# do-mpc/do-mpc

Measured on AMD Instinct MI355X. Metric: MPC steps/sec (make_step wall-time), industrial_poly robust multi-stage, higher is better.
Workload: dtype f64

## Files before the change

### do_mpc_amd/csrc/dompc_driver.h

```cpp

DOMPC_DEV inline int epsg_off(const KArgs& A) { return A.node_eps_off[0]; }
DOMPC_DEV inline int epsg_n(const KArgs& A) { return A.n_opt_x - A.node_eps_off[0]; }
DOMPC_DEV inline void epsg_grad(const Thr& T, const Prob& Q) {
  const KArgs& A = *Q.A;
  const int o = epsg_off(A), nv = epsg_n(A);
  for (int j = T.tid; j < nv; j += T.nt) {
    double g = 0.0, r = 0.0;
    for (int e = 0; e < A.n_edges; ++e) {
      const int q = j - (A.node_eps_off[A.edge_parent[e]] - o);
      if (q < 0 || q >= NSE) continue;
      g += Q.sf * DOMPC_EPS_PEN[q];
      const double* yd = Q.lam + A.edge_row0[e] + NW + NX;
      for (int i = 0; i < NE; ++i)
        if (nl_slack(i) == q) r -= yd[i] * Q.sgn[e * NE1 + i];
    }
    Q.gf[o + j] = g;
    Q.rd[o + j] = g + r - Q.zl[o + j] + Q.zu[o + j];
  }
  T.sync();
}
DOMPC_DEV inline double epsg_rowsum(const Prob& Q, int j, const double* v, const double* v0) {
  const KArgs& A = *Q.A;
  const int o = epsg_off(A);
  double t = 0.0;
// ... 10 lines not shown
  const KArgs& A = *Q.A;
  const int o = epsg_off(A);
  for (int e = T.tid; e < A.n_edges; e += T.nt) {
    const int jo = A.node_eps_off[A.edge_parent[e]] - o;
    const int r0 = A.edge_row0[e] + NW + NX;
    for (int i = 0; i < NE; ++i) {
      const int q = nl_slack(i);
      if (q < 0) continue;
      const double ve = v ? v[jo + q] : ((jo + q == j1) ? 1.0 : 0.0);
      Q.c[r0 + i] = Q.ct[r0 + i] - ve * Q.sgn[e * NE1 + i];
    }
  }
  T.sync();
}

DOMPC_DEV inline void solve_problem(const Thr& T, const KArgs& A, int b, int slot) {
  const dompc_options& O = A.opt;
  Prob Q = make_prob(A, slot, A.p + (int64_t)b * A.n_opt_p);
  const double* x0 = A.x0 + (int64_t)b * A.n_opt_x;
  const int nX = A.n_opt_x, nSl = A.n_edges * NE;
  int status = 2, it = 0, n_reg = 0, n_ls_fail = 0, n_sweeps = 0, n_trials = 0, n_soc = 0;

  double cnt[2] = {0.0, 0.0};
  bool singular0;
  {
    double fr[1] = {0.0};
    for (int d = T.tid; d < A.n_dummy; d += T.nt) {
      const int g = A.dummy_idx[d];
      if (!(A.lbx[g] > -INFINITY) && !(A.ubx[g] < INFINITY)) fr[0] += 1.0;
    }
    const int ops[1] = {R_SUM};
    wg_reduce(T, fr, ops);
// ... 247 lines not shown
    if (KAPPA_D != 0.0) bs[0] += KAPPA_D * lin;
    const int ops[1] = {R_SUM};
    wg_reduce(T, bs, ops);
    bar_sum = bs[0];
  }
  int n_filt = 0;
  double delta_last = 0.0;
  int acc_count = 0;
  const double s_max = 100.0;
  double E0 = 0.0;
  int wd_count = 0, wd_iter = 0, n_watchdog = 0;
  bool in_wd = false, wd_resume = false;
  double wd_theta = 0.0, wd_phi = 0.0, wd_dphi = 0.0, wd_alpha = 0.0, wd_amax = 0.0, wd_az = 0.0, wd_delta = 0.0, wd_delta_last = 0.0, wd_bar = 0.0;
  Errs wd_E = E;
  double delta = 0.0, a_max = 1.0, a_z = 1.0, dphi = 0.0;

  while (true) {
    bool skip_first = false;
    if (wd_resume) {
      for (int g = T.tid; g < nX; g += T.nt) { Q.x[g] = Q.x_wd[g]; Q.zl[g] = Q.zl_wd[g]; Q.zu[g] = Q.zu_wd[g]; Q.dx[g] = Q.dx_sv[g]; }
      for (int g = T.tid; g < A.n_g; g += T.nt) { Q.lam[g] = Q.lam_wd[g]; Q.dlam[g] = Q.dlam_sv[g]; }
      for (int g = T.tid; g < nSl; g += T.nt) { Q.s[g] = Q.s_wd[g]; Q.zsl[g] = Q.zsl_wd[g]; Q.zsu[g] = Q.zsu_wd[g]; Q.ds[g] = Q.ds_sv[g]; }
      T.sync();
      E = wd_E; bar_sum = wd_bar; delta = wd_delta; delta_last = wd_delta_last; a_max = wd_amax; a_z = wd_az; dphi = wd_dphi;
      wd_resume = false;
      skip_first = true;
    } else {
    if (bad) { if (in_wd) { bad = 0; wd_resume = true; in_wd = false; wd_count = 0; continue; } status = 3; break; }
    if (T.fget(6)) { status = 6; break; }
    if (((WIDE_OK && T.nwg > 1) || sh_on(A)) && T.fget(7)) { status = 5; break; }
// ... 72 lines not shown
    auto step_rules = [&](double (&r5)[5]) { run_step_rules(T, Q, b, slot, mu, r5); };
    const double theta = E.theta;
    const double phi = E.obj + mu * bar_sum;

    c_t = prof_clock(); g_t = T.gen;
    const double gamma_theta = 1e-5, gamma_phi = 1e-8, eta_phi = 1e-8, s_theta = 1.1, s_phi = 2.3, gamma_alpha = 0.05;
    const double kappa_soc = 0.99;
    double a_min;
    if (dphi < 0.0 && theta <= theta_min)
      a_min = (theta > 0.0) ? gamma_alpha * fmin(gamma_theta, fmin(gamma_phi * theta / (-dphi),
                                                                    pow(theta, s_theta) / pow(-dphi, s_phi)))
                            : gamma_alpha * gamma_theta;
    else if (dphi < 0.0) a_min = gamma_alpha * fmin(gamma_theta, gamma_phi * theta / (-dphi));
    else a_min = gamma_alpha * gamma_theta;
    a_min = fmax(a_min, 1e-14);
    auto eval_trial = [&](double al, double& obj_o, double& th_o, double& bar_o) {
      run_eval_trial(T, Q, b, slot, al, obj_o, th_o, bar_o);
      ++n_trials;
    };
    auto acceptable_ref = [&](double th_, double ph_, double al, bool& armijo_case, double theta, double phi, double dphi) -> bool {
      armijo_case = false;
      bool ok = (ph_ == ph_) && (th_ == th_) && fabs(ph_) < INFINITY && th_ <= theta_max;
      if (ok) {
        for (int q = 0; q < n_filt; ++q)
          if (th_ >= T.filt[2 * q] && ph_ >= T.filt[2 * q + 1]) { ok = false; break; }
      }
      if (ok) {
        const bool switching = dphi < 0.0 && al * pow(-dphi, s_phi) > pow(theta, s_theta);
        const double eps_m = 10.0 * 2.220446049250313e-16 * fabs(phi);
        if (theta <= theta_min && switching) {
          armijo_case = true;
          ok = (ph_ - phi - eps_m <= eta_phi * al * dphi);
// ... 22 lines not shown
    double alpha = skip_first ? 0.5 * a_max : a_max;
    bool accepted = false, armijo_used = false, stale = false;
    double th_t = 0.0, obj_t = 0.0, bar_t = bar_sum;
    int n_ls = skip_first ? 1 : 0;
    bool wd_done = false, wd_augment_ref = false, wd_no_augment = false;
    if (O.watchdog_shortened_iter_trigger > 0 && !in_wd && !skip_first && wd_count >= O.watchdog_shortened_iter_trigger) {
      in_wd = true; wd_iter = 0; ++n_watchdog;
      for (int g = T.tid; g < nX; g += T.nt) { Q.x_wd[g] = Q.x[g]; Q.zl_wd[g] = Q.zl[g]; Q.zu_wd[g] = Q.zu[g]; Q.dx_sv[g] = Q.dx[g]; }
      for (int g = T.tid; g < A.n_g; g += T.nt) { Q.lam_wd[g] = Q.lam[g]; Q.dlam_sv[g] = Q.dlam[g]; }
      for (int g = T.tid; g < nSl; g += T.nt) { Q.s_wd[g] = Q.s[g]; Q.zsl_wd[g] = Q.zsl[g]; Q.zsu_wd[g] = Q.zsu[g]; Q.ds_sv[g] = Q.ds[g]; }
      T.sync();
      wd_E = E; wd_bar = bar_sum; wd_delta = delta; wd_delta_last = delta_last; wd_amax = a_max; wd_az = a_z;
      wd_theta = theta; wd_phi = phi; wd_dphi = dphi; wd_alpha = a_max;
    }
    if (in_wd) {
      eval_trial(alpha, obj_t, th_t, bar_t);
      bool armijo_case = false;
      if (acceptable_ref(th_t, obj_t + mu * bar_t, wd_alpha, armijo_case, wd_theta, wd_phi, wd_dphi)) {
        accepted = true; armijo_used = armijo_case; wd_done = true; wd_augment_ref = true;
        in_wd = false; wd_count = 0;
      } else {
        ++wd_iter;
        const double ph_ = obj_t + mu * bar_t;
        if (wd_iter > O.watchdog_trial_iter_max || !(ph_ == ph_) || !(th_t == th_t) || !(fabs(ph_) < INFINITY)) {
          wd_resume = true; in_wd = false; wd_count = 0;
          continue;
        }
        accepted = true; wd_done = true; wd_no_augment = true;
      }
    }
    while (!wd_done) {
      eval_trial(alpha, obj_t, th_t, bar_t);
      stale = false;
      bool armijo_case = false;
      if (acceptable(th_t, obj_t + mu * bar_t, alpha, armijo_case)) { accepted = true; armijo_used = armijo_case; break; }
      if (n_ls == 0 && O.max_soc > 0 && th_t >= theta) {
        double th_old = theta;
        keep_direction(false);
        soc_residual(alpha);
        bool soc_ok = false;
        for (int k = 0; k < O.max_soc; ++k) {
          ++n_soc; ++n_sweeps;
          if (run_sweep(T, Q, b, slot, mu, 1, delta)) break;
          if (run_backward(T, Q, b, slot, mu, delta)) break;
          run_forward(T, Q, b, slot, mu, delta);
          if (EPS_GLOBAL && epsg_apply(delta, Q.dlam)) break;
          double q5[5];
          step_rules(q5);
          const double a_s = (q5[0] > tau) ? tau / q5[0] : 1.0;
          double obj_s = 0.0, th_s = 0.0, bar_s = 0.0;
          eval_trial(a_s, obj_s, th_s, bar_s);
          bool arm_s = false;
          if (acceptable(th_s, obj_s + mu * bar_s, a_s, arm_s)) {
            accepted = true; armijo_used = arm_s; soc_ok = true;
            alpha = a_s;
            a_z = (q5[1] > tau) ? tau / q5[1] : 1.0;
            obj_t = obj_s; th_t = th_s; bar_t = bar_s;
            break;
          }
          if (!(th_s <= kappa_soc * th_old)) break;
          th_old = th_s;
          soc_residual(a_s);
        }
        if (soc_ok) break;
        keep_direction(true);
        stale = true;
      }
      if (!(alpha * 0.5 >= a_min)) break;
      alpha *= 0.5;
      ++n_ls;
    }
    if (bad) { if (in_wd) { bad = 0; wd_resume = true; in_wd = false; wd_count = 0; continue; } status = 3; break; }
    if (!accepted && stale) eval_trial(alpha, obj_t, th_t, bar_t);
    if (!wd_done) wd_count = n_ls > 0 ? wd_count + 1 : 0;
    if (!accepted) {
      ++n_ls_fail;
      n_filt = 0;
    } else if (!armijo_used && !wd_no_augment) {
      if (T.ltid == 0) {
        int q = n_filt < MAX_FILTER ? n_filt : MAX_FILTER - 1;
        T.filt[2 * q] = (1.0 - gamma_theta) * (wd_augment_ref ? wd_theta : theta);
        T.filt[2 * q + 1] = (wd_augment_ref ? wd_phi : phi) - gamma_phi * (wd_augment_ref ? wd_theta : theta);
      }
      if (n_filt < MAX_FILTER) ++n_filt;
      T.lsync();
    }
    bar_sum = bar_t;
    c_ls += prof_clock() - c_t; g_ls += T.gen - g_t;
    c_t = prof_clock(); g_t = T.gen;
    const Comp Cp = run_accept(T, Q, b, slot, alpha, a_z, mu);
    if (A.trace && b == 0 && T.tid == 0 && it < A.trace_cap) {
      double* tr = A.trace + 8 * it;
      tr[0] = it; tr[1] = mu; tr[2] = E0; tr[3] = E.e_p; tr[4] = E.e_d; tr[5] = accepted ? alpha : -alpha;
      tr[6] = delta; tr[7] = E.obj / Q.sf;
    }
    if (T.tid == 0) T.fset(6, abort_requested(A));
    T.sync();
    c_acc += prof_clock() - c_t; g_acc += T.gen - g_t;
    ++it;
    c_t = prof_clock(); g_t = T.gen; bad = run_sweep(T, Q, b, slot, mu, 0, singular0 ? delta_after(delta_last) : 0.0); c_sweep += prof_clock() - c_t; g_sweep += T.gen - g_t;
    ++n_sweeps;
    if (EPS_GLOBAL) epsg_grad(T, Q);
    if (KAPPA_D != 0.0) Q.mu = mu;
    c_t = prof_clock(); g_t = T.gen; E = measure(T, Q, &Cp); c_meas += prof_clock() - c_t; g_meas += T.gen - g_t;
  }

  if (A.trace && b == 0 && T.tid == 0 && A.trace_cap > 8) { double* tr = A.trace + 8 * (A.trace_cap - 1); tr[0] = (double)c_sweep; tr[1] = (double)c_bwd; tr[2] = (double)c_fwd; tr[3] = (double)c_ls; tr[4] = (double)c_meas; tr[5] = (double)(prof_clock() - c_start); tr[6] = (double)c_ftb; tr[7] = (double)c_acc; if (T.prof) { double* t2 = A.trace + 8 * (A.trace_cap - 2); for (int i = 0; i < 8; ++i) t2[i] = (double)T.prof[i]; double* t3 = A.trace + 8 * (A.trace_cap - 3); for (int i = 0; i < 8; ++i) t3[i] = (double)T.prof[8 + i]; double* t4 = A.trace + 8 * (A.trace_cap - 4); for (int i = 0; i < 8; ++i) t4[i] = (double)T.prof[16 + i]; if (A.trace_cap > 12) { double* t5 = A.trace + 8 * (A.trace_cap - 5); for (int i = 0; i < 8; ++i) t5[i] = (double)T.prof[24 + i]; double* t6 = A.trace + 8 * (A.trace_cap - 6); t6[0] = g_sweep; t6[1] = g_bwd; t6[2] = g_fwd; t6[3] = g_ls; t6[4] = g_meas; t6[5] = T.gen - g_start; t6[6] = g_ftb; t6[7] = g_acc; } } }
  const double isf = 1.0 / Q.sf;
  if (A.x_out) for (int g = T.tid; g < nX; g += T.nt) A.x_out[(int64_t)b * nX + g] = sh_cnt(A, mk_x(A, g)) ? Q.x[g] : 0.0;
  if (A.lam_x_out) for (int g = T.tid; g < nX; g += T.nt) A.lam_x_out[(int64_t)b * nX + g] = sh_cnt(A, mk_x(A, g)) ? (Q.zu[g] - Q.zl[g]) * isf : 0.0;
  if (A.lam_g_out) for (int r = T.tid; r < A.n_g; r += T.nt) A.lam_g_out[(int64_t)b * A.n_g + r] = sh_cnt(A, mk_g(A, r)) ? Q.lam[r] * isf : 0.0;
  if (A.lam_g_out && NE > 0) {
    T.sync();
    for (int g = T.tid; g < nSl; g += T.nt) {
      const int e = g / NE1, i = g % NE1;
      if (!sh_cnt(A, mk_e(A, e))) continue;
      const int row = A.edge_row0[e] + NW + NX + i;
      A.lam_g_out[(int64_t)b * A.n_g + row] = Q.lam[row] * Q.sgn[e * NE1 + i] * isf;
    }
  }
  if (A.g_out) {
// ... 112 lines not shown
```

### do_mpc_amd/csrc/dompc_kernel.h

```cpp
#pragma once
#include <math.h>
#include <stdint.h>
#ifndef DOMPC_HOST_EMU
#include <utility>
#endif
#include "dompc_kargs.h"

namespace dompc {

#ifndef DOMPC_HOST_EMU
#define DOMPC_PHASE __device__ inline
#else
#define DOMPC_PHASE static inline
#endif

constexpr int NX = DOMPC_NX, NU = DOMPC_NU, NP = DOMPC_NP, NTVP = DOMPC_NTVP;
#ifndef DOMPC_EPS_GLOBAL
#define DOMPC_EPS_GLOBAL 0
#endif
constexpr bool EPS_GLOBAL = DOMPC_EPS_GLOBAL != 0 && DOMPC_NS > 0 && DOMPC_NE > 0;
constexpr int NS = EPS_GLOBAL ? 0 : DOMPC_NS;
constexpr int NSE = DOMPC_NS;
constexpr int NVG_MAX = 32;
constexpr int NZ = DOMPC_NZ;
// ... 107 lines not shown
constexpr int ND_P = 0;
constexpr int ND_PV = ND_P + NA * NA;
constexpr int ND_K = ND_PV + NA;
constexpr int ND_KV = ND_K + NV * NA;
constexpr int ND_DXT = ND_KV + NV;
constexpr int ND_AT = ND_DXT + NA;
constexpr int AT_LEN = FREE_ROOT ? 1 + NX + NX * NX : 0;
constexpr int ND_SIZE = ((ND_AT + AT_LEN + 7) / 8) * 8;

struct WsLayout {
  int64_t x, zl, zu, lb, ub, dx, gf, rd, xt, dx_sv;
  int64_t lam, dlam, c, ct, dlam_sv;
  int64_t s, zsl, zsu, sl, su, ds, st, ds_sv;
  int64_t ew, es, nd, mo, gsc, total;
  int64_t x_wd, zl_wd, zu_wd, lam_wd, s_wd, zsl_wd, zsu_wd, dlam_e, sgn;
};

DOMPC_HD inline WsLayout ws_layout(int n_opt_x, int n_g, int n_edges, int e_pad, int n_nodes) {
  WsLayout L;
  int64_t o = 0;
  auto take = [&](int64_t n) { int64_t r = o; o += (n + 7) & ~int64_t(7); return r; };
  L.x = take(n_opt_x); L.zl = take(n_opt_x); L.zu = take(n_opt_x); L.lb = take(n_opt_x); L.ub = take(n_opt_x);
  L.dx = take(n_opt_x); L.gf = take(n_opt_x); L.rd = take(n_opt_x); L.xt = take(n_opt_x);
  L.dx_sv = take(n_opt_x);
  L.lam = take(n_g); L.dlam = take(n_g); L.c = take(n_g); L.ct = take(n_g); L.dlam_sv = take(n_g);
  int64_t nsl = (int64_t)n_edges * NE1;
  L.s = take(nsl); L.zsl = take(nsl); L.zsu = take(nsl); L.sl = take(nsl); L.su = take(nsl);
  L.ds = take(nsl); L.st = take(nsl); L.ds_sv = take(nsl);
  L.ew = take((int64_t)EW_SIZE * e_pad);
  L.es = take((int64_t)ES_SIZE * n_edges);
  L.nd = take((int64_t)ND_SIZE * n_nodes);
  L.mo = take((int64_t)MO_REC * n_edges);
  L.gsc = take(EPS_GLOBAL ? NVG_MAX * (NVG_MAX + 4) : 0);
  L.x_wd = take(n_opt_x); L.zl_wd = take(n_opt_x); L.zu_wd = take(n_opt_x); L.lam_wd = take(n_g);
  L.s_wd = take(nsl); L.zsl_wd = take(nsl); L.zsu_wd = take(nsl);
  L.dlam_e = take(EPS_GLOBAL ? n_g : 0);
  L.sgn = take(nsl);
  o += 256;
  L.total = o;
  return L;
}

#ifndef DOMPC_HOST_EMU
typedef __attribute__((address_space(3))) double ldsd;
#else
typedef double ldsd;
#endif

struct XCtx {
  int on, rank, world;
  double* xbuf;
  volatile uint32_t *req, *ack, *cnt;
// ... 307 lines not shown
    for (int l = 0; l < k; ++l) t += A[i * sai + l * sal] * B[l * sbl + j * sbj];
    D[i * ldd + j] = (beta == 0.0) ? t : beta * D[i * ldd + j] + t;
  }
#endif
}

struct Prob {
  const KArgs* A;
  const double* P;
  double *x, *zl, *zu, *lb, *ub, *dx, *gf, *rd, *xt, *dx_sv;
  double *lb_own, *ub_own;
  double *lam, *dlam, *c, *ct, *dlam_sv;
  double *s, *zsl, *zsu, *sl, *su, *ds, *st, *ds_sv;
  double *ew, *es, *nd, *mo, *gsc;
  double *x_wd, *zl_wd, *zu_wd, *lam_wd, *s_wd, *zsl_wd, *zsu_wd, *dlam_e, *sgn;
  int e_pad;
  double sf;
  double mu;
  int soc;
  double dsw;
  int slot;
  int rp_soc; double rp_mu;
  int lu_ok;
  DOMPC_DEV double& EW(int e, int i) const { return ew[(int64_t)e * EW_SIZE + i]; }
  DOMPC_DEV double* ES(int e) const { return es + (int64_t)e * ES_SIZE; }
  DOMPC_DEV double* ND(int n) const { return nd + (int64_t)n * ND_SIZE; }
  DOMPC_DEV double* MO(int e) const { return mo + (int64_t)e * MO_REC; }
};

DOMPC_DEV inline Prob make_prob(const KArgs& A, int slot, const double* P) {
  WsLayout L = ws_layout(A.n_opt_x, A.n_g, A.n_edges, A.e_pad, A.n_nodes);
  double* w = A.ws + (int64_t)slot * A.ws_stride;
  Prob p;
  p.A = &A; p.P = P;
  p.x = w + L.x; p.zl = w + L.zl; p.zu = w + L.zu; p.lb_own = w + L.lb; p.ub_own = w + L.ub; p.dx = w + L.dx;
  p.lb = A.lb_sh ? A.lb_sh : p.lb_own; p.ub = A.ub_sh ? A.ub_sh : p.ub_own;
  p.gf = w + L.gf; p.rd = w + L.rd; p.xt = w + L.xt; p.dx_sv = w + L.dx_sv;
  p.lam = w + L.lam; p.dlam = w + L.dlam; p.c = w + L.c; p.ct = w + L.ct; p.dlam_sv = w + L.dlam_sv;
  p.s = w + L.s; p.zsl = w + L.zsl; p.zsu = w + L.zsu; p.sl = w + L.sl; p.su = w + L.su;
  p.ds = w + L.ds; p.st = w + L.st; p.ds_sv = w + L.ds_sv;
  p.ew = w + L.ew; p.es = w + L.es; p.nd = w + L.nd; p.mo = w + L.mo; p.gsc = w + L.gsc;
  p.x_wd = w + L.x_wd; p.zl_wd = w + L.zl_wd; p.zu_wd = w + L.zu_wd; p.lam_wd = w + L.lam_wd;
  p.s_wd = w + L.s_wd; p.zsl_wd = w + L.zsl_wd; p.zsu_wd = w + L.zsu_wd; p.dlam_e = w + L.dlam_e; p.sgn = w + L.sgn;
  p.e_pad = A.e_pad; p.sf = 1.0; p.mu = 0.0; p.soc = 0; p.dsw = 0.0; p.slot = slot; p.lu_ok = 1; p.rp_soc = 0; p.rp_mu = 0.0;
  return p;
}
DOMPC_DEV inline void prob_bounds(Prob& Q) {
  const KArgs& A = *Q.A;
  const bool own = (Q.soc & 2) != 0 || !A.lb_sh;
  Q.lb = own ? Q.lb_own : A.lb_sh;
  Q.ub = own ? Q.ub_own : A.ub_sh;
}

DOMPC_DEV constexpr int slot_of(int i, int r) { return i == 0 ? r - 1 : DEG + (i - 1) * (DEG + 1) + r; }
DOMPC_DEV constexpr int next_slot(int i) { return (i + 1 < NI) ? slot_of(i + 1, 0) : M - 1; }

DOMPC_DEV inline int group_index(int tid, int gs) {
#ifndef DOMPC_HOST_EMU
  return __builtin_amdgcn_readfirstlane(tid / gs);
// ... 139 lines not shown
```

### do_mpc_amd/csrc/dompc_phases.h

```cpp

template <bool FINE>
DOMPC_DEV inline double trial_edges(const Thr& T, const Prob& Q) {
  const KArgs& A = *Q.A;
  double f = 0.0;
  if (FINE && !DENSE_EDGE && M > 0) {
    constexpr int NPC = NI * DEG + 1;
    for (int it = T.tid; it < A.n_edges * NPC; it += T.nt) {
      const int e = it % A.n_edges, q = it / A.n_edges;
      const double fe = eval_edge_f_t<true>(Q, e, Q.xt, Q.st, Q.ct, q == 0 ? NI * DEG : q - 1);
      f += fe;
    }
  } else
  for (int e = T.tid; e < A.n_edges; e += T.nt) {
    const int m = mk_e(A, e);
    if (!m) continue;
    const double fe = DENSE_EDGE ? dae_edge_f(Q, e, Q.xt, Q.st, Q.ct) : eval_edge_f(Q, e, Q.xt, Q.st, Q.ct);
    if (sh_cnt(A, m)) f += fe;
  }
  for (int n = T.tid; n < A.n_nodes; n += T.nt)
    if (sh_cnt(A, mk_n(A, n))) f += node_rterm_f(Q, n, Q.xt);
  return f;
}
DOMPC_DEV inline void step_rules_pass(const Thr& T, const Prob& Q, double mu, double (&r5)[5]) {
  const KArgs& A = *Q.A;
// ... 37 lines not shown
      gphi -= mu * r;
    }
    if (u < INFINITY) {
      const double r = fast_rcp(u - sv);
      r5[0] = fmax(r5[0], d * r);
      r5[1] = fmax(r5[1], 1.0 - r * d - mu * r * fast_rcp(Q.zsu[si]));
      gphi += mu * r;
    }
    if (KAPPA_D != 0.0) gphi += KAPPA_D * mu * one_sided(l, u);
    r5[2] += gphi * d;
  }
  const int ops[5] = {R_MAX, R_MAX, R_SUM, R_SUM, R_SUM};
  wg_reduce(T, r5, ops);
}
template <bool FINE>
DOMPC_DEV inline void eval_trial_pass(const Thr& T, const Prob& Q, double al, double& obj_o, double& th_o, double& bar_o) {
  const KArgs& A = *Q.A;
  const int nX = A.n_opt_x, nSl = A.n_edges * NE;
  double r3[3] = {0.0, 0.0, 0.0};
  LogAcc La{1.0, 0, 0};
  double lin = 0.0;
  {
    double x_[DOMPC_FW], d_[DOMPC_FW], l_[DOMPC_FW], u2_[DOMPC_FW];
#define L_(u, g) x_[u] = Q.x[g]; d_[u] = Q.dx[g]; l_[u] = Q.lb[g]; u2_[u] = Q.ub[g];
#define B_(u, g)                                                                               \
    if (mk_x(A, g)) {                                                                      \
      const double xt_ = x_[u] + al * d_[u];                                               \
      Q.xt[g] = xt_;                                                                       \
      if (sh_cnt(A, mk_x(A, g))) {                                                         \
        if (l_[u] > -INFINITY) logacc_add(La, xt_ - l_[u]);                                \
        if (u2_[u] < INFINITY) logacc_add(La, u2_[u] - xt_);                               \
        if (KAPPA_D != 0.0) { const double os_ = one_sided(l_[u], u2_[u]); lin += os_ > 0.0 ? xt_ - l_[u] : (os_ < 0.0 ? u2_[u] - xt_ : 0.0); } \
      }                                                                                    \
    }
    DOMPC_FOR4(nX, L_, B_)
#undef L_
#undef B_
  }
  for (int g = T.tid; g < nSl; g += T.nt) {
    if (!mk_e(A, g / NE1)) continue;
    const int si = (g / NE1) * NE1 + g % NE1;
    Q.st[si] = Q.s[si] + al * Q.ds[si];
  }
  T.sync();
  for (int g = T.tid; g < NX; g += T.nt) Q.ct[g] = FREE_ROOT ? 0.0 : Q.xt[A.node_x_off[0] + g] - Q.P[g] / DOMPC_SX[g];
  if (FREE_ROOT && T.tid == 0) r3[0] += Q.sf * dompc_aterm_f(Q.xt + A.node_x_off[0], Q.P, Q.P + A.p_off_tvp, Q.P + A.p_off_p);
  r3[0] += trial_edges<FINE>(T, Q);
  T.sync();
  {
    double c_[DOMPC_FW];
#define L_(u, g) c_[u] = Q.ct[g];
#define B_(u, g) if (sh_cnt(A, mk_g(A, g))) r3[1] += fabs(c_[u]);
    DOMPC_FOR4(A.n_g, L_, B_)
#undef L_
#undef B_
  }
  for (int g = T.tid; g < nSl; g += T.nt) {
    if (!sh_cnt(A, mk_e(A, g / NE1))) continue;
    const int si = (g / NE1) * NE1 + g % NE1;
    if (Q.sl[si] > -INFINITY) logacc_add(La, Q.st[si] - Q.sl[si]);
    if (Q.su[si] < INFINITY) logacc_add(La, Q.su[si] - Q.st[si]);
    if (KAPPA_D != 0.0) { const double os_ = one_sided(Q.sl[si], Q.su[si]); lin += os_ > 0.0 ? Q.st[si] - Q.sl[si] : (os_ < 0.0 ? Q.su[si] - Q.st[si] : 0.0); }
  }
  r3[2] = -logacc_value(La);
  if (KAPPA_D != 0.0) r3[2] += KAPPA_D * lin;
  const int ops[3] = {R_SUM, R_SUM, R_SUM};
  wg_reduce(T, r3, ops);
  obj_o = r3[0]; th_o = r3[1]; bar_o = r3[2];
}
DOMPC_DEV inline Comp accept_pass(const Thr& T, const Prob& Q, double alpha, double a_z, double mu) {
  const KArgs& A = *Q.A;
  const int nX = A.n_opt_x, nSl = A.n_edges * NE;
  const double ks = 1e10;
  Comp Cp{-INFINITY, INFINITY, 0.0};
  {
    double xt_[DOMPC_FW], x_[DOMPC_FW], d_[DOMPC_FW], l_[DOMPC_FW], u2_[DOMPC_FW], zl_[DOMPC_FW], zu_[DOMPC_FW];
#define L_(u, g) xt_[u] = Q.xt[g]; x_[u] = Q.x[g]; d_[u] = Q.dx[g]; l_[u] = Q.lb[g]; u2_[u] = Q.ub[g]; zl_[u] = Q.zl[g]; zu_[u] = Q.zu[g];
#define B_(u, g)                                                                               \
    if (mk_x(A, g)) {                                                                        \
      const double xv = xt_[u], l = l_[u], ub_ = u2_[u];                                     \
      const bool cnt_ = sh_cnt(A, mk_x(A, g));                                               \
      Q.x[g] = xv;                                                                           \
      if (l > -INFINITY) {                                                                   \
        const double ro = fast_rcp(x_[u] - l);                       \
        const double z = zl_[u] + a_z * (mu * ro - zl_[u] - zl_[u] * ro * d_[u]);            \
        const double dd = xv - l, mr = mu * fast_rcp(dd);                                    \
        const double zn = fmax(fmin(z, ks * mr), mr * (1.0 / ks));                           \
        Q.zl[g] = zn;                                                                        \
        if (cnt_) comp_add(Cp, dd * zn, zn);                                                 \
      }                                                                                      \
      if (ub_ < INFINITY) {                                                                  \
        const double ro = fast_rcp(ub_ - x_[u]);                                             \
        const double z = zu_[u] + a_z * (mu * ro - zu_[u] + zu_[u] * ro * d_[u]);            \
        const double dd = ub_ - xv, mr = mu * fast_rcp(dd);                                  \
        const double zn = fmax(fmin(z, ks * mr), mr * (1.0 / ks));                           \
        Q.zu[g] = zn;                                                                        \
        if (cnt_) comp_add(Cp, dd * zn, zn);                                                 \
      }                                                                                      \
    }
    DOMPC_FOR4(nX, L_, B_)
#undef L_
#undef B_
  }
  for (int g = T.tid; g < nSl; g += T.nt) {
    if (!mk_e(A, g / NE1)) continue;
    const int si = (g / NE1) * NE1 + g % NE1;
    const double sv = Q.st[si], so = Q.s[si], dsv = Q.ds[si];
    const bool cnt_ = sh_cnt(A, mk_e(A, g / NE1));
    Q.s[si] = sv;
    const double l = Q.sl[si], u = Q.su[si];
    if (l > -INFINITY) {
      const double z = Q.zsl[si] + a_z * dz_lo(so, l, Q.zsl[si], dsv, mu);
      const double zn = fmax(fmin(z, ks * mu / (sv - l)), mu / (ks * (sv - l)));
      Q.zsl[si] = zn;
      if (cnt_) comp_add(Cp, (sv - l) * zn, zn);
    }
    if (u < INFINITY) {
      const double z = Q.zsu[si] + a_z * dz_up(so, u, Q.zsu[si], dsv, mu);
      const double zn = fmax(fmin(z, ks * mu / (u - sv)), mu / (ks * (u - sv)));
      Q.zsu[si] = zn;
      if (cnt_) comp_add(Cp, (u - sv) * zn, zn);
    }
  }
  {
    double y_[DOMPC_FW], dy_[DOMPC_FW];
#define L_(u, g) y_[u] = Q.lam[g]; dy_[u] = Q.dlam[g];
#define B_(u, g) if (mk_g(A, g)) Q.lam[g] = y_[u] + alpha * dy_[u];
    DOMPC_FOR4(A.n_g, L_, B_)
#undef L_
#undef B_
  }
  return Cp;
}
struct PhaseRet { unsigned gen, nred, xseq; int rc; };
struct PhaseRet3 { unsigned gen, nred, xseq; double v0, v1, v2; };
#ifndef DOMPC_HOST_EMU
#define DOMPC_PHASE_PROLOGUE                                                        \
  const KArgs A = kernel_args(kp);                                                  \
  Thr T = make_thr(A);                                                              \
  T.kp = kp;                                                                        \
  T.gen = ufl(gen); T.nred = ufl(nred); T.xseq = ufl(xseq);                         \
  Prob Q = make_prob(A, ufl(slot), A.p + (int64_t)ufl(b) * A.n_opt_p);              \
  Q.sf = ufl(sf);
__device__ __attribute__((noinline)) PhaseRet phase_sweep(const void* kp, int b, int slot, double sf, double mu, double dsw, int soc, unsigned gen, unsigned nred, unsigned xseq) {
  DOMPC_PHASE_PROLOGUE
  Q.soc = ufl(soc);
  prob_bounds(Q);
  Q.dsw = ufl(dsw);
  const int rc = sweep<false>(T, Q, ufl(mu));
  return PhaseRet{T.gen, T.nred, T.xseq, rc};
// ... 20 lines not shown
  riccati_forward_t<false>(T, Q, ufl(mu), ufl(delta));
  return PhaseRet{T.gen, T.nred, T.xseq, 0};
}
__device__ __attribute__((noinline)) PhaseRet phase_forward_adj(const void* kp, int b, int slot, double sf, double mu, double delta, double dsw, unsigned gen, unsigned nred, unsigned xseq) {
  DOMPC_PHASE_PROLOGUE
  Q.dsw = ufl(dsw);
  riccati_forward_t<true>(T, Q, ufl(mu), ufl(delta));
  return PhaseRet{T.gen, T.nred, T.xseq, 0};
}
__device__ __attribute__((noinline)) PhaseRet3 phase_step_rules(const void* kp, int b, int slot, double sf, double mu, unsigned gen, unsigned nred, unsigned xseq) {
  DOMPC_PHASE_PROLOGUE
  double r5[5];
  step_rules_pass(T, Q, ufl(mu), r5);
  return PhaseRet3{T.gen, T.nred, T.xseq, r5[0], r5[1], r5[2]};
}
__device__ __attribute__((noinline)) PhaseRet3 phase_eval_trial(const void* kp, int b, int slot, double sf, double al, unsigned gen, unsigned nred, unsigned xseq) {
  DOMPC_PHASE_PROLOGUE
  double o = 0.0, th = 0.0, br = 0.0;
  eval_trial_pass<false>(T, Q, ufl(al), o, th, br);
  return PhaseRet3{T.gen, T.nred, T.xseq, o, th, br};
}
__device__ __attribute__((noinline)) PhaseRet3 phase_eval_trial_fine(const void* kp, int b, int slot, double sf, double al, unsigned gen, unsigned nred, unsigned xseq) {
  DOMPC_PHASE_PROLOGUE
  double o = 0.0, th = 0.0, br = 0.0;
  eval_trial_pass<true>(T, Q, ufl(al), o, th, br);
  return PhaseRet3{T.gen, T.nred, T.xseq, o, th, br};
}
__device__ __attribute__((noinline)) PhaseRet3 phase_accept(const void* kp, int b, int slot, double sf, double alpha, double a_z, double mu, unsigned gen, unsigned nred, unsigned xseq) {
  DOMPC_PHASE_PROLOGUE
  const Comp C = accept_pass(T, Q, ufl(alpha), ufl(a_z), ufl(mu));
  return PhaseRet3{T.gen, T.nred, T.xseq, C.smax, C.smin, C.sum_z};
}
#undef DOMPC_PHASE_PROLOGUE
#define DOMPC_PHASE_CALL(fn, ...)                                                   \
  const auto r_ = fn(T.kp, b, slot, Q.sf, __VA_ARGS__, T.gen, T.nred, T.xseq);            \
  T.gen = ufl(r_.gen); T.nred = ufl(r_.nred); T.xseq = ufl(r_.xseq);
#endif
#ifndef DOMPC_REPEAT_PHASE
#define DOMPC_REPEAT_PHASE 0
#endif
DOMPC_DEV inline int run_sweep(const Thr& T, Prob& Q, int b, int slot, double mu, int soc = 0, double dsw = 0.0) {
  Q.dsw = dsw;
  Q.lu_ok = lu_store_rule(*Q.A, mu, soc) ? 1 : 0;
  Q.rp_soc = soc; Q.rp_mu = mu;
#ifndef DOMPC_HOST_EMU
  if (fine_items(T, *Q.A)) { DOMPC_PHASE_CALL(phase_sweep_fine, mu, dsw, soc) return ufl(r_.rc); }
// ... 24 lines not shown
  Qm.soc = mode;
  prob_bounds(Qm);
  return riccati_backward(T, Qm, mu, delta);
#endif
}
DOMPC_DEV inline void run_step_rules(const Thr& T, const Prob& Q, int b, int slot, double mu, double (&r5)[5]) {
#ifndef DOMPC_HOST_EMU
  if (DOMPC_REPEAT_PHASE & 16) { DOMPC_PHASE_CALL(phase_step_rules, mu) }
  DOMPC_PHASE_CALL(phase_step_rules, mu)
  r5[0] = ufl(r_.v0); r5[1] = ufl(r_.v1); r5[2] = ufl(r_.v2); r5[3] = 0.0; r5[4] = 0.0;
#else
  (void)b; (void)slot;
  step_rules_pass(T, Q, mu, r5);
#endif
}
DOMPC_DEV inline void run_eval_trial(const Thr& T, const Prob& Q, int b, int slot, double al, double& obj_o, double& th_o, double& bar_o) {
#ifndef DOMPC_HOST_EMU
  if (fine_items(T, *Q.A)) { DOMPC_PHASE_CALL(phase_eval_trial_fine, al) obj_o = ufl(r_.v0); th_o = ufl(r_.v1); bar_o = ufl(r_.v2); return; }
  if (DOMPC_REPEAT_PHASE & 8) { DOMPC_PHASE_CALL(phase_eval_trial, al) }
  DOMPC_PHASE_CALL(phase_eval_trial, al)
  obj_o = ufl(r_.v0); th_o = ufl(r_.v1); bar_o = ufl(r_.v2);
#else
  (void)b; (void)slot;
  if (fine_items(T, *Q.A)) eval_trial_pass<true>(T, Q, al, obj_o, th_o, bar_o); else eval_trial_pass<false>(T, Q, al, obj_o, th_o, bar_o);
#endif
}
DOMPC_DEV inline Comp run_accept(const Thr& T, const Prob& Q, int b, int slot, double alpha, double a_z, double mu) {
#ifndef DOMPC_HOST_EMU
  DOMPC_PHASE_CALL(phase_accept, alpha, a_z, mu)
  return Comp{r_.v0, r_.v1, r_.v2};
#else
  (void)b; (void)slot;
  return accept_pass(T, Q, alpha, a_z, mu);
#endif
}
DOMPC_DEV inline void run_forward(const Thr& T, const Prob& Q, int b, int slot, double mu, double delta) {
#ifndef DOMPC_HOST_EMU
  if (forward_adjoint(Q, mu)) {
    DOMPC_PHASE_CALL(phase_forward_adj, mu, delta, Q.dsw)
  } else {
    if (DOMPC_REPEAT_PHASE & 4) { DOMPC_PHASE_CALL(phase_forward, mu, delta, Q.dsw) }
    DOMPC_PHASE_CALL(phase_forward, mu, delta, Q.dsw)
  }
#else
  (void)b; (void)slot;
  if (forward_adjoint(Q, mu)) riccati_forward_t<true>(T, Q, mu, delta);
  else riccati_forward_t<false>(T, Q, mu, delta);
#endif
// ... 4 lines not shown
```

Measured before the change: 10190.

## Fuse accept pass into trial evaluation with double-buffered iterate swap

Trial evaluation now also computes trial dual variables (zl, zu, zsl, zsu) and multipliers into shadow buffers, along with the complementarity stats. Acceptance becomes a pointer swap between current and trial buffers instead of a separate accept phase with its own memory pass and sync. This removes one full read/write sweep and one phase call per iteration. The cost is extra dual work and extra workspace on every line-search trial, including rejected ones, plus parity tracking through the slot index.

```diff
diff --git a/do_mpc_amd/csrc/dompc_driver.h b/do_mpc_amd/csrc/dompc_driver.h
--- a/do_mpc_amd/csrc/dompc_driver.h
+++ b/do_mpc_amd/csrc/dompc_driver.h
@@ -48,8 +48,9 @@
   T.sync();
 }
 
-DOMPC_DEV inline void solve_problem(const Thr& T, const KArgs& A, int b, int slot) {
+DOMPC_DEV inline void solve_problem(const Thr& T, const KArgs& A, int b, int slot0) {
   const dompc_options& O = A.opt;
+  int slot = slot0;
   Prob Q = make_prob(A, slot, A.p + (int64_t)b * A.n_opt_p);
   const double* x0 = A.x0 + (int64_t)b * A.n_opt_x;
   const int nX = A.n_opt_x, nSl = A.n_edges * NE;
@@ -327,6 +328,11 @@
   double wd_theta = 0.0, wd_phi = 0.0, wd_dphi = 0.0, wd_alpha = 0.0, wd_amax = 0.0, wd_az = 0.0, wd_delta = 0.0, wd_delta_last = 0.0, wd_bar = 0.0;
   Errs wd_E = E;
   double delta = 0.0, a_max = 1.0, a_z = 1.0, dphi = 0.0;
+  for (int g = T.tid; g < nX; g += T.nt) { Q.xt[g] = Q.x[g]; Q.zlt[g] = Q.zl[g]; Q.zut[g] = Q.zu[g]; }
+  for (int g = T.tid; g < A.n_g; g += T.nt) Q.lamt[g] = Q.lam[g];
+  for (int g = T.tid; g < nSl; g += T.nt) { Q.st[g] = Q.s[g]; Q.zslt[g] = Q.zsl[g]; Q.zsut[g] = Q.zsu[g]; }
+  T.sync();
+  Comp Cp{-INFINITY, INFINITY, 0.0};
 
   while (true) {
     bool skip_first = false;
@@ -429,8 +435,8 @@
     else if (dphi < 0.0) a_min = gamma_alpha * fmin(gamma_theta, gamma_phi * theta / (-dphi));
     else a_min = gamma_alpha * gamma_theta;
     a_min = fmax(a_min, 1e-14);
-    auto eval_trial = [&](double al, double& obj_o, double& th_o, double& bar_o) {
-      run_eval_trial(T, Q, b, slot, al, obj_o, th_o, bar_o);
+    auto eval_trial = [&](double al, double az, double& obj_o, double& th_o, double& bar_o) {
+      run_eval_trial(T, Q, b, slot, al, az, mu, obj_o, th_o, bar_o, Cp);
       ++n_trials;
     };
     auto acceptable_ref = [&](double th_, double ph_, double al, bool& armijo_case, double theta, double phi, double dphi) -> bool {
@@ -483,7 +489,7 @@
       wd_theta = theta; wd_phi = phi; wd_dphi = dphi; wd_alpha = a_max;
     }
     if (in_wd) {
-      eval_trial(alpha, obj_t, th_t, bar_t);
+      eval_trial(alpha, a_z, obj_t, th_t, bar_t);
       bool armijo_case = false;
       if (acceptable_ref(th_t, obj_t + mu * bar_t, wd_alpha, armijo_case, wd_theta, wd_phi, wd_dphi)) {
         accepted = true; armijo_used = armijo_case; wd_done = true; wd_augment_ref = true;
@@ -499,7 +505,7 @@
       }
     }
     while (!wd_done) {
-      eval_trial(alpha, obj_t, th_t, bar_t);
+      eval_trial(alpha, a_z, obj_t, th_t, bar_t);
       stale = false;
       bool armijo_case = false;
       if (acceptable(th_t, obj_t + mu * bar_t, alpha, armijo_case)) { accepted = true; armijo_used = armijo_case; break; }
@@ -517,13 +523,14 @@
           double q5[5];
           step_rules(q5);
           const double a_s = (q5[0] > tau) ? tau / q5[0] : 1.0;
+          const double az_s = (q5[1] > tau) ? tau / q5[1] : 1.0;
           double obj_s = 0.0, th_s = 0.0, bar_s = 0.0;
-          eval_trial(a_s, obj_s, th_s, bar_s);
+          eval_trial(a_s, az_s, obj_s, th_s, bar_s);
           bool arm_s = false;
           if (acceptable(th_s, obj_s + mu * bar_s, a_s, arm_s)) {
             accepted = true; armijo_used = arm_s; soc_ok = true;
             alpha = a_s;
-            a_z = (q5[1] > tau) ? tau / q5[1] : 1.0;
+            a_z = az_s;
             obj_t = obj_s; th_t = th_s; bar_t = bar_s;
             break;
           }
@@ -540,7 +547,7 @@
       ++n_ls;
     }
     if (bad) { if (in_wd) { bad = 0; wd_resume = true; in_wd = false; wd_count = 0; continue; } status = 3; break; }
-    if (!accepted && stale) eval_trial(alpha, obj_t, th_t, bar_t);
+    if (!accepted && stale) eval_trial(alpha, a_z, obj_t, th_t, bar_t);
     if (!wd_done) wd_count = n_ls > 0 ? wd_count + 1 : 0;
     if (!accepted) {
       ++n_ls_fail;
@@ -557,14 +564,13 @@
     bar_sum = bar_t;
     c_ls += prof_clock() - c_t; g_ls += T.gen - g_t;
     c_t = prof_clock(); g_t = T.gen;
-    const Comp Cp = run_accept(T, Q, b, slot, alpha, a_z, mu);
+    prob_flip(Q); slot = Q.slot;
     if (A.trace && b == 0 && T.tid == 0 && it < A.trace_cap) {
       double* tr = A.trace + 8 * it;
       tr[0] = it; tr[1] = mu; tr[2] = E0; tr[3] = E.e_p; tr[4] = E.e_d; tr[5] = accepted ? alpha : -alpha;
       tr[6] = delta; tr[7] = E.obj / Q.sf;
     }
     if (T.tid == 0) T.fset(6, abort_requested(A));
-    T.sync();
     c_acc += prof_clock() - c_t; g_acc += T.gen - g_t;
     ++it;
     c_t = prof_clock(); g_t = T.gen; bad = run_sweep(T, Q, b, slot, mu, 0, singular0 ? delta_after(delta_last) : 0.0); c_sweep += prof_clock() - c_t; g_sweep += T.gen - g_t;
@@ -574,6 +580,13 @@
     c_t = prof_clock(); g_t = T.gen; E = measure(T, Q, &Cp); c_meas += prof_clock() - c_t; g_meas += T.gen - g_t;
   }
 
+  if (slot & SLOT_PARITY) {
+    for (int g = T.tid; g < nX; g += T.nt) { Q.xt[g] = Q.x[g]; Q.zlt[g] = Q.zl[g]; Q.zut[g] = Q.zu[g]; }
+    for (int g = T.tid; g < A.n_g; g += T.nt) Q.lamt[g] = Q.lam[g];
+    for (int g = T.tid; g < nSl; g += T.nt) { Q.st[g] = Q.s[g]; Q.zslt[g] = Q.zsl[g]; Q.zsut[g] = Q.zsu[g]; }
+    T.sync();
+    prob_flip(Q); slot = Q.slot;
+  }
   if (A.trace && b == 0 && T.tid == 0 && A.trace_cap > 8) { double* tr = A.trace + 8 * (A.trace_cap - 1); tr[0] = (double)c_sweep; tr[1] = (double)c_bwd; tr[2] = (double)c_fwd; tr[3] = (double)c_ls; tr[4] = (double)c_meas; tr[5] = (double)(prof_clock() - c_start); tr[6] = (double)c_ftb; tr[7] = (double)c_acc; if (T.prof) { double* t2 = A.trace + 8 * (A.trace_cap - 2); for (int i = 0; i < 8; ++i) t2[i] = (double)T.prof[i]; double* t3 = A.trace + 8 * (A.trace_cap - 3); for (int i = 0; i < 8; ++i) t3[i] = (double)T.prof[8 + i]; double* t4 = A.trace + 8 * (A.trace_cap - 4); for (int i = 0; i < 8; ++i) t4[i] = (double)T.prof[16 + i]; if (A.trace_cap > 12) { double* t5 = A.trace + 8 * (A.trace_cap - 5); for (int i = 0; i < 8; ++i) t5[i] = (double)T.prof[24 + i]; double* t6 = A.trace + 8 * (A.trace_cap - 6); t6[0] = g_sweep; t6[1] = g_bwd; t6[2] = g_fwd; t6[3] = g_ls; t6[4] = g_meas; t6[5] = T.gen - g_start; t6[6] = g_ftb; t6[7] = g_acc; } } }
   const double isf = 1.0 / Q.sf;
   if (A.x_out) for (int g = T.tid; g < nX; g += T.nt) A.x_out[(int64_t)b * nX + g] = sh_cnt(A, mk_x(A, g)) ? Q.x[g] : 0.0;
diff --git a/do_mpc_amd/csrc/dompc_kernel.h b/do_mpc_amd/csrc/dompc_kernel.h
--- a/do_mpc_amd/csrc/dompc_kernel.h
+++ b/do_mpc_amd/csrc/dompc_kernel.h
@@ -145,6 +145,7 @@
   int64_t s, zsl, zsu, sl, su, ds, st, ds_sv;
   int64_t ew, es, nd, mo, gsc, total;
   int64_t x_wd, zl_wd, zu_wd, lam_wd, s_wd, zsl_wd, zsu_wd, dlam_e, sgn;
+  int64_t zlt, zut, lamt, zslt, zsut;
 };
 
 DOMPC_HD inline WsLayout ws_layout(int n_opt_x, int n_g, int n_edges, int e_pad, int n_nodes) {
@@ -167,6 +168,7 @@
   L.s_wd = take(nsl); L.zsl_wd = take(nsl); L.zsu_wd = take(nsl);
   L.dlam_e = take(EPS_GLOBAL ? n_g : 0);
   L.sgn = take(nsl);
+  L.zlt = take(n_opt_x); L.zut = take(n_opt_x); L.lamt = take(n_g); L.zslt = take(nsl); L.zsut = take(nsl);
   o += 256;
   L.total = o;
   return L;
@@ -504,6 +506,7 @@
   double *s, *zsl, *zsu, *sl, *su, *ds, *st, *ds_sv;
   double *ew, *es, *nd, *mo, *gsc;
   double *x_wd, *zl_wd, *zu_wd, *lam_wd, *s_wd, *zsl_wd, *zsu_wd, *dlam_e, *sgn;
+  double *zlt, *zut, *lamt, *zslt, *zsut;
   int e_pad;
   double sf;
   double mu;
@@ -518,9 +521,16 @@
   DOMPC_DEV double* MO(int e) const { return mo + (int64_t)e * MO_REC; }
 };
 
+constexpr int SLOT_PARITY = 1 << 30;
+template <class T_> DOMPC_DEV inline void swap_ptr(T_*& a, T_*& b) { T_* t = a; a = b; b = t; }
+DOMPC_DEV inline void prob_flip(Prob& p) {
+  swap_ptr(p.x, p.xt); swap_ptr(p.zl, p.zlt); swap_ptr(p.zu, p.zut); swap_ptr(p.lam, p.lamt);
+  swap_ptr(p.s, p.st); swap_ptr(p.zsl, p.zslt); swap_ptr(p.zsu, p.zsut);
+  p.slot ^= SLOT_PARITY;
+}
 DOMPC_DEV inline Prob make_prob(const KArgs& A, int slot, const double* P) {
   WsLayout L = ws_layout(A.n_opt_x, A.n_g, A.n_edges, A.e_pad, A.n_nodes);
-  double* w = A.ws + (int64_t)slot * A.ws_stride;
+  double* w = A.ws + (int64_t)(slot & ~SLOT_PARITY) * A.ws_stride;
   Prob p;
   p.A = &A; p.P = P;
   p.x = w + L.x; p.zl = w + L.zl; p.zu = w + L.zu; p.lb_own = w + L.lb; p.ub_own = w + L.ub; p.dx = w + L.dx;
@@ -532,7 +542,9 @@
   p.ew = w + L.ew; p.es = w + L.es; p.nd = w + L.nd; p.mo = w + L.mo; p.gsc = w + L.gsc;
   p.x_wd = w + L.x_wd; p.zl_wd = w + L.zl_wd; p.zu_wd = w + L.zu_wd; p.lam_wd = w + L.lam_wd;
   p.s_wd = w + L.s_wd; p.zsl_wd = w + L.zsl_wd; p.zsu_wd = w + L.zsu_wd; p.dlam_e = w + L.dlam_e; p.sgn = w + L.sgn;
-  p.e_pad = A.e_pad; p.sf = 1.0; p.mu = 0.0; p.soc = 0; p.dsw = 0.0; p.slot = slot; p.lu_ok = 1; p.rp_soc = 0; p.rp_mu = 0.0;
+  p.zlt = w + L.zlt; p.zut = w + L.zut; p.lamt = w + L.lamt; p.zslt = w + L.zslt; p.zsut = w + L.zsut;
+  p.e_pad = A.e_pad; p.sf = 1.0; p.mu = 0.0; p.soc = 0; p.dsw = 0.0; p.slot = slot & ~SLOT_PARITY; p.lu_ok = 1; p.rp_soc = 0; p.rp_mu = 0.0;
+  if (slot & SLOT_PARITY) prob_flip(p);
   return p;
 }
 DOMPC_DEV inline void prob_bounds(Prob& Q) {
diff --git a/do_mpc_amd/csrc/dompc_phases.h b/do_mpc_amd/csrc/dompc_phases.h
--- a/do_mpc_amd/csrc/dompc_phases.h
+++ b/do_mpc_amd/csrc/dompc_phases.h
@@ -75,24 +75,44 @@
   wg_reduce(T, r5, ops);
 }
 template <bool FINE>
-DOMPC_DEV inline void eval_trial_pass(const Thr& T, const Prob& Q, double al, double& obj_o, double& th_o, double& bar_o) {
+DOMPC_DEV inline void eval_trial_pass(const Thr& T, const Prob& Q, double al, double a_z, double mu, double& obj_o, double& th_o, double& bar_o, Comp& Cp) {
   const KArgs& A = *Q.A;
   const int nX = A.n_opt_x, nSl = A.n_edges * NE;
+  const double ks = 1e10;
   double r3[3] = {0.0, 0.0, 0.0};
   LogAcc La{1.0, 0, 0};
   double lin = 0.0;
+  Cp = Comp{-INFINITY, INFINITY, 0.0};
   {
-    double x_[DOMPC_FW], d_[DOMPC_FW], l_[DOMPC_FW], u2_[DOMPC_FW];
-#define L_(u, g) x_[u] = Q.x[g]; d_[u] = Q.dx[g]; l_[u] = Q.lb[g]; u2_[u] = Q.ub[g];
+    double x_[DOMPC_FW], d_[DOMPC_FW], l_[DOMPC_FW], u2_[DOMPC_FW], zl_[DOMPC_FW], zu_[DOMPC_FW];
+#define L_(u, g) x_[u] = Q.x[g]; d_[u] = Q.dx[g]; l_[u] = Q.lb[g]; u2_[u] = Q.ub[g]; zl_[u] = Q.zl[g]; zu_[u] = Q.zu[g];
 #define B_(u, g)                                                                               \
     if (mk_x(A, g)) {                                                                      \
       const double xt_ = x_[u] + al * d_[u];                                               \
+      const double xv = xt_, l = l_[u], ub_ = u2_[u];                                      \
+      const bool cnt_ = sh_cnt(A, mk_x(A, g));                                             \
       Q.xt[g] = xt_;                                                                       \
-      if (sh_cnt(A, mk_x(A, g))) {                                                         \
+      if (cnt_) {                                                                          \
         if (l_[u] > -INFINITY) logacc_add(La, xt_ - l_[u]);                                \
         if (u2_[u] < INFINITY) logacc_add(La, u2_[u] - xt_);                               \
         if (KAPPA_D != 0.0) { const double os_ = one_sided(l_[u], u2_[u]); lin += os_ > 0.0 ? xt_ - l_[u] : (os_ < 0.0 ? u2_[u] - xt_ : 0.0); } \
       }                                                                                    \
+      if (l > -INFINITY) {                                                                 \
+        const double ro = fast_rcp(x_[u] - l);                       \
+        const double z = zl_[u] + a_z * (mu * ro - zl_[u] - zl_[u] * ro * d_[u]);          \
+        const double dd = xv - l, mr = mu * fast_rcp(dd);                                  \
+        const double zn = fmax(fmin(z, ks * mr), mr * (1.0 / ks));                         \
+        Q.zlt[g] = zn;                                                                     \
+        if (cnt_) comp_add(Cp, dd * zn, zn);                                               \
+      }                                                                                    \
+      if (ub_ < INFINITY) {                                                                \
+        const double ro = fast_rcp(ub_ - x_[u]);                                           \
+        const double z = zu_[u] + a_z * (mu * ro - zu_[u] + zu_[u] * ro * d_[u]);          \
+        const double dd = ub_ - xv, mr = mu * fast_rcp(dd);                                \
+        const double zn = fmax(fmin(z, ks * mr), mr * (1.0 / ks));                         \
+        Q.zut[g] = zn;                                                                     \
+        if (cnt_) comp_add(Cp, dd * zn, zn);                                               \
+      }                                                                                    \
     }
     DOMPC_FOR4(nX, L_, B_)
 #undef L_
@@ -101,7 +121,31 @@
   for (int g = T.tid; g < nSl; g += T.nt) {
     if (!mk_e(A, g / NE1)) continue;
     const int si = (g / NE1) * NE1 + g % NE1;
-    Q.st[si] = Q.s[si] + al * Q.ds[si];
+    const double so = Q.s[si], dsv = Q.ds[si];
+    const double sv = so + al * dsv;
+    const bool cnt_ = sh_cnt(A, mk_e(A, g / NE1));
+    Q.st[si] = sv;
+    const double l = Q.sl[si], u = Q.su[si];
+    if (l > -INFINITY) {
+      const double z = Q.zsl[si] + a_z * dz_lo(so, l, Q.zsl[si], dsv, mu);
+      const double zn = fmax(fmin(z, ks * mu / (sv - l)), mu / (ks * (sv - l)));
+      Q.zslt[si] = zn;
+      if (cnt_) comp_add(Cp, (sv - l) * zn, zn);
+    }
+    if (u < INFINITY) {
+      const double z = Q.zsu[si] + a_z * dz_up(so, u, Q.zsu[si], dsv, mu);
+      const double zn = fmax(fmin(z, ks * mu / (u - sv)), mu / (ks * (u - sv)));
+      Q.zsut[si] = zn;
+      if (cnt_) comp_add(Cp, (u - sv) * zn, zn);
+    }
+  }
+  {
+    double y_[DOMPC_FW], dy_[DOMPC_FW];
+#define L_(u, g) y_[u] = Q.lam[g]; dy_[u] = Q.dlam[g];
+#define B_(u, g) if (mk_g(A, g)) Q.lamt[g] = y_[u] + al * dy_[u];
+    DOMPC_FOR4(A.n_g, L_, B_)
+#undef L_
+#undef B_
   }
   T.sync();
   for (int g = T.tid; g < NX; g += T.nt) Q.ct[g] = FREE_ROOT ? 0.0 : Q.xt[A.node_x_off[0] + g] - Q.P[g] / DOMPC_SX[g];
@@ -129,72 +173,9 @@
   wg_reduce(T, r3, ops);
   obj_o = r3[0]; th_o = r3[1]; bar_o = r3[2];
 }
-DOMPC_DEV inline Comp accept_pass(const Thr& T, const Prob& Q, double alpha, double a_z, double mu) {
-  const KArgs& A = *Q.A;
-  const int nX = A.n_opt_x, nSl = A.n_edges * NE;
-  const double ks = 1e10;
-  Comp Cp{-INFINITY, INFINITY, 0.0};
-  {
-    double xt_[DOMPC_FW], x_[DOMPC_FW], d_[DOMPC_FW], l_[DOMPC_FW], u2_[DOMPC_FW], zl_[DOMPC_FW], zu_[DOMPC_FW];
-#define L_(u, g) xt_[u] = Q.xt[g]; x_[u] = Q.x[g]; d_[u] = Q.dx[g]; l_[u] = Q.lb[g]; u2_[u] = Q.ub[g]; zl_[u] = Q.zl[g]; zu_[u] = Q.zu[g];
-#define B_(u, g)                                                                               \
-    if (mk_x(A, g)) {                                                                        \
-      const double xv = xt_[u], l = l_[u], ub_ = u2_[u];                                     \
-      const bool cnt_ = sh_cnt(A, mk_x(A, g));                                               \
-      Q.x[g] = xv;                                                                           \
-      if (l > -INFINITY) {                                                                   \
-        const double ro = fast_rcp(x_[u] - l);                       \
-        const double z = zl_[u] + a_z * (mu * ro - zl_[u] - zl_[u] * ro * d_[u]);            \
-        const double dd = xv - l, mr = mu * fast_rcp(dd);                                    \
-        const double zn = fmax(fmin(z, ks * mr), mr * (1.0 / ks));                           \
-        Q.zl[g] = zn;                                                                        \
-        if (cnt_) comp_add(Cp, dd * zn, zn);                                                 \
-      }                                                                                      \
-      if (ub_ < INFINITY) {                                                                  \
-        const double ro = fast_rcp(ub_ - x_[u]);                                             \
-        const double z = zu_[u] + a_z * (mu * ro - zu_[u] + zu_[u] * ro * d_[u]);            \
-        const double dd = ub_ - xv, mr = mu * fast_rcp(dd);                                  \
-        const double zn = fmax(fmin(z, ks * mr), mr * (1.0 / ks));                           \
-        Q.zu[g] = zn;                                                                        \
-        if (cnt_) comp_add(Cp, dd * zn, zn);                                                 \
-      }                                                                                      \
-    }
-    DOMPC_FOR4(nX, L_, B_)
-#undef L_
-#undef B_
-  }
-  for (int g = T.tid; g < nSl; g += T.nt) {
-    if (!mk_e(A, g / NE1)) continue;
-    const int si = (g / NE1) * NE1 + g % NE1;
-    const double sv = Q.st[si], so = Q.s[si], dsv = Q.ds[si];
-    const bool cnt_ = sh_cnt(A, mk_e(A, g / NE1));
-    Q.s[si] = sv;
-    const double l = Q.sl[si], u = Q.su[si];
-    if (l > -INFINITY) {
-      const double z = Q.zsl[si] + a_z * dz_lo(so, l, Q.zsl[si], dsv, mu);
-      const double zn = fmax(fmin(z, ks * mu / (sv - l)), mu / (ks * (sv - l)));
-      Q.zsl[si] = zn;
-      if (cnt_) comp_add(Cp, (sv - l) * zn, zn);
-    }
-    if (u < INFINITY) {
-      const double z = Q.zsu[si] + a_z * dz_up(so, u, Q.zsu[si], dsv, mu);
-      const double zn = fmax(fmin(z, ks * mu / (u - sv)), mu / (ks * (u - sv)));
-      Q.zsu[si] = zn;
-      if (cnt_) comp_add(Cp, (u - sv) * zn, zn);
-    }
-  }
-  {
-    double y_[DOMPC_FW], dy_[DOMPC_FW];
-#define L_(u, g) y_[u] = Q.lam[g]; dy_[u] = Q.dlam[g];
-#define B_(u, g) if (mk_g(A, g)) Q.lam[g] = y_[u] + alpha * dy_[u];
-    DOMPC_FOR4(A.n_g, L_, B_)
-#undef L_
-#undef B_
-  }
-  return Cp;
-}
 struct PhaseRet { unsigned gen, nred, xseq; int rc; };
 struct PhaseRet3 { unsigned gen, nred, xseq; double v0, v1, v2; };
+struct PhaseRet6 { unsigned gen, nred, xseq; double v0, v1, v2, c0, c1, c2; };
 #ifndef DOMPC_HOST_EMU
 #define DOMPC_PHASE_PROLOGUE                                                        \
   const KArgs A = kernel_args(kp);                                                  \
@@ -245,22 +226,19 @@
   step_rules_pass(T, Q, ufl(mu), r5);
   return PhaseRet3{T.gen, T.nred, T.xseq, r5[0], r5[1], r5[2]};
 }
-__device__ __attribute__((noinline)) PhaseRet3 phase_eval_trial(const void* kp, int b, int slot, double sf, double al, unsigned gen, unsigned nred, unsigned xseq) {
+__device__ __attribute__((noinline)) PhaseRet6 phase_eval_trial(const void* kp, int b, int slot, double sf, double al, double a_z, double mu, unsigned gen, unsigned nred, unsigned xseq) {
   DOMPC_PHASE_PROLOGUE
   double o = 0.0, th = 0.0, br = 0.0;
-  eval_trial_pass<false>(T, Q, ufl(al), o, th, br);
-  return PhaseRet3{T.gen, T.nred, T.xseq, o, th, br};
-}
-__device__ __attribute__((noinline)) PhaseRet3 phase_eval_trial_fine(const void* kp, int b, int slot, double sf, double al, unsigned gen, unsigned nred, unsigned xseq) {
+  Comp C;
+  eval_trial_pass<false>(T, Q, ufl(al), ufl(a_z), ufl(mu), o, th, br, C);
+  return PhaseRet6{T.gen, T.nred, T.xseq, o, th, br, C.smax, C.smin, C.sum_z};
+}
+__device__ __attribute__((noinline)) PhaseRet6 phase_eval_trial_fine(const void* kp, int b, int slot, double sf, double al, double a_z, double mu, unsigned gen, unsigned nred, unsigned xseq) {
   DOMPC_PHASE_PROLOGUE
   double o = 0.0, th = 0.0, br = 0.0;
-  eval_trial_pass<true>(T, Q, ufl(al), o, th, br);
-  return PhaseRet3{T.gen, T.nred, T.xseq, o, th, br};
-}
-__device__ __attribute__((noinline)) PhaseRet3 phase_accept(const void* kp, int b, int slot, double sf, double alpha, double a_z, double mu, unsigned gen, unsigned nred, unsigned xseq) {
-  DOMPC_PHASE_PROLOGUE
-  const Comp C = accept_pass(T, Q, ufl(alpha), ufl(a_z), ufl(mu));
-  return PhaseRet3{T.gen, T.nred, T.xseq, C.smax, C.smin, C.sum_z};
+  Comp C;
+  eval_trial_pass<true>(T, Q, ufl(al), ufl(a_z), ufl(mu), o, th, br, C);
+  return PhaseRet6{T.gen, T.nred, T.xseq, o, th, br, C.smax, C.smin, C.sum_z};
 }
 #undef DOMPC_PHASE_PROLOGUE
 #define DOMPC_PHASE_CALL(fn, ...)                                                   \
@@ -315,24 +293,15 @@
   step_rules_pass(T, Q, mu, r5);
 #endif
 }
-DOMPC_DEV inline void run_eval_trial(const Thr& T, const Prob& Q, int b, int slot, double al, double& obj_o, double& th_o, double& bar_o) {
-#ifndef DOMPC_HOST_EMU
-  if (fine_items(T, *Q.A)) { DOMPC_PHASE_CALL(phase_eval_trial_fine, al) obj_o = ufl(r_.v0); th_o = ufl(r_.v1); bar_o = ufl(r_.v2); return; }
-  if (DOMPC_REPEAT_PHASE & 8) { DOMPC_PHASE_CALL(phase_eval_trial, al) }
-  DOMPC_PHASE_CALL(phase_eval_trial, al)
-  obj_o = ufl(r_.v0); th_o = ufl(r_.v1); bar_o = ufl(r_.v2);
-#else
-  (void)b; (void)slot;
-  if (fine_items(T, *Q.A)) eval_trial_pass<true>(T, Q, al, obj_o, th_o, bar_o); else eval_trial_pass<false>(T, Q, al, obj_o, th_o, bar_o);
-#endif
-}
-DOMPC_DEV inline Comp run_accept(const Thr& T, const Prob& Q, int b, int slot, double alpha, double a_z, double mu) {
-#ifndef DOMPC_HOST_EMU
-  DOMPC_PHASE_CALL(phase_accept, alpha, a_z, mu)
-  return Comp{r_.v0, r_.v1, r_.v2};
-#else
-  (void)b; (void)slot;
-  return accept_pass(T, Q, alpha, a_z, mu);
+DOMPC_DEV inline void run_eval_trial(const Thr& T, const Prob& Q, int b, int slot, double al, double a_z, double mu, double& obj_o, double& th_o, double& bar_o, Comp& Cp) {
+#ifndef DOMPC_HOST_EMU
+  if (fine_items(T, *Q.A)) { DOMPC_PHASE_CALL(phase_eval_trial_fine, al, a_z, mu) obj_o = ufl(r_.v0); th_o = ufl(r_.v1); bar_o = ufl(r_.v2); Cp = Comp{r_.c0, r_.c1, r_.c2}; return; }
+  if (DOMPC_REPEAT_PHASE & 8) { DOMPC_PHASE_CALL(phase_eval_trial, al, a_z, mu) }
+  DOMPC_PHASE_CALL(phase_eval_trial, al, a_z, mu)
+  obj_o = ufl(r_.v0); th_o = ufl(r_.v1); bar_o = ufl(r_.v2); Cp = Comp{r_.c0, r_.c1, r_.c2};
+#else
+  (void)b; (void)slot;
+  if (fine_items(T, *Q.A)) eval_trial_pass<true>(T, Q, al, a_z, mu, obj_o, th_o, bar_o, Cp); else eval_trial_pass<false>(T, Q, al, a_z, mu, obj_o, th_o, bar_o, Cp);
 #endif
 }
 DOMPC_DEV inline void run_forward(const Thr& T, const Prob& Q, int b, int slot, double mu, double delta) {
```

Measured after the change: 10770, median of 6. +5.7%, better.
